# WISDEM/RAFT

Hardware: NVIDIA H100
Metric: RAO solves/sec (freq-bins x cases x designs) (higher is better)
Workload: dtype f64

## Files before the change

raft_b200/csrc/raftk.cu:

```cuda
#include <cuda_runtime.h>
#include <cooperative_groups.h>
#include <math_constants.h>
#include <stdint.h>
#include <stdio.h>
#include <stdlib.h>
#include <string.h>
#include <mutex>
#include <algorithm>
#include <type_traits>
#include <vector>

#include "../../include/raftk.h"

namespace cg = cooperative_groups;

static thread_local char g_err[512] = "";
static long long g_launches = 0;

static int set_err(int code, const char *fmt, const char *a = "", const char *b = "")
{
    snprintf(g_err, sizeof(g_err), fmt, a, b);
    return code;
}
#define CUDA_TRY(expr)                                                                          \
// ... 430 lines not shown
    CUDA_TRY(cudaOccupancyMaxActiveClusters(&clusters, k_rao_fused2<false>, &cfg));
    CUDA_TRY(cudaOccupancyMaxActiveBlocksPerMultiprocessor(&per_sm, k_rao_fused2<true>, F2_T, pl.smem));
    resident = per_sm * sm_count();
    std::lock_guard<std::mutex> lk(g_f2_occ_mu);
    g_f2_occ.push_back(F2Occ{dev, units, pl.CS, pl.smem, clusters, resident});
    return RAFTK_OK;
}

static int f2_pick_grid(const SolvePlan &pl, int units, bool &grid)
{
    grid = false;
    const char *x = getenv("RAFTK_FUSED2_XCHG");
    const bool force_c = x && !strcmp(x, "cluster"), force_g = x && !strcmp(x, "grid");
    if (x && *x && !force_c && !force_g) return set_err(RAFTK_EINVAL, "RAFTK_FUSED2_XCHG must be 'cluster' or 'grid', not '%s'", x);
    if (pl.CS <= 1 || force_c) return RAFTK_OK;
    int clusters = 0, resident = 0;
    if (int rc = f2_occupancy(pl, units, clusters, resident)) return rc;
    const bool fits = pl.xslots && (size_t)units * pl.CS <= (size_t)resident;
    if (force_g && !fits) return set_err(RAFTK_EINVAL, "RAFTK_FUSED2_XCHG=grid: the launch's CTAs cannot all be resident at once");
    grid = fits && (force_g || clusters < units);
    return RAFTK_OK;
}

static int run_fused2(const raftk_designs *d, const raftk_cases *c, const raftk_solve_opts *o, const raftk_outputs *out,
                      const SolvePlan &pl, void *workspace, cudaStream_t st, const raftk_peers *peers)
{
    prof_begin_call();
    DesignsDev D = to_dev(d, d->max_nodes, d->max_members);
    CasesDev C = to_dev(c);
    char *ws = static_cast<char *>(workspace);
    FusedParams P = fused_params(d, c, o, out, pl, peers);
    P.F0g = reinterpret_cast<double2 *>(ws);
    P.Eg = reinterpret_cast<double2 *>(ws + pl.o_E);
    P.Ag = reinterpret_cast<double2 *>(ws + pl.o_A);
    double *plan = reinterpret_cast<double *>(ws + pl.o_plan);
    P.plan = plan; P.plan_stride = pl.blob;
    if (!(o->flags & RAFTK_SOLVE_REUSE_PLAN)) {
        ProfScope ps(st, 0);
        const size_t psm = (3 * (size_t)d->max_nodes + d->max_members) * sizeof(double) + 2 * (size_t)d->max_members * sizeof(int);
        k_fused_plan<<<d->n_designs, 128, psm, st>>>(D, plan, pl.blob, pl.maxW, pl.maxH, pl.maxZ, pl.nwl);
        g_launches++;
    }
    const int units = d->n_designs * c->n_cases;
    bool grid = false;
    if (int rc = f2_pick_grid(pl, units, grid)) return rc;
    CUDA_TRY(grid ? g_f2_opt_grid.ensure(k_rao_fused2<true>, pl.smem) : g_f2_opt_cluster.ensure(k_rao_fused2<false>, pl.smem));
    cudaLaunchConfig_t cfg;
    cudaLaunchAttribute at;
    cluster_config(cfg, at, (size_t)units * pl.CS, F2_T, pl.smem, pl.CS, st);
    if (grid) {
        at.id = cudaLaunchAttributeCooperative;
        at.val.cooperative = 1;
        P.xrow = reinterpret_cast<double *>(ws + pl.o_xrow);
        P.xcnt = reinterpret_cast<unsigned *>(ws + pl.o_xcnt);
    }
    const int nphase = c->primary ? 2 : 1;
    if (c->primary) P.lin_g = reinterpret_cast<double *>(ws + pl.o_lin);
    for (int phase = 0; phase < nphase; phase++) {
        P.phase = c->primary ? phase : -1;
        {
            ProfScope ps(st, 2);
            if (grid) {
                CUDA_TRY(cudaMemsetAsync(P.xcnt, 0, (size_t)units * sizeof(unsigned), st));
                CUDA_TRY(cudaLaunchKernelEx(&cfg, k_rao_fused2<true>, D, C, P));
            } else {
                CUDA_TRY(cudaLaunchKernelEx(&cfg, k_rao_fused2<false>, D, C, P));
            }
        }
        g_launches++;
    }
    disp_launch(RAFTK_FAMILY_SOLVE, grid ? RAFTK_KERNEL_FUSED2_GRID : RAFTK_KERNEL_FUSED2_CLUSTER, F2_T, pl.CS, pl.nwl);
    g_disp.trains = c->primary != nullptr;
    CUDA_TRY(cudaGetLastError());
    return RAFTK_OK;
}

#ifdef RAFTK_F2_WAVE_TRACE
extern "C" int raftk_f2_trace_read(unsigned long long *host, int n_cta)
{
    if (n_cta < 0 || n_cta > F2_TRACE_MAX) return set_err(RAFTK_EINVAL, "n_cta must be in [0, F2_TRACE_MAX]");
    CUDA_TRY(cudaMemcpyFromSymbol(host, g_f2_trace, (size_t)n_cta * 3 * sizeof(unsigned long long)));
    return RAFTK_OK;
}
extern "C" int raftk_f2_occupancy(const raftk_designs *d, int n_cases, int cluster_size, int out[5])
{
    const SolvePlan pl = plan_solve(d, n_cases, cluster_size, WS_UNBOUNDED);
    if (pl.kind != SOLVE_FUSED2) return set_err(RAFTK_EINVAL, "not a k_rao_fused2 shape");
    const int units = d->n_designs * n_cases;
    int clusters = 0, resident = 0;
    bool grid = false;
    if (int rc = f2_occupancy(pl, units, clusters, resident)) return rc;
    if (int rc = f2_pick_grid(pl, units, grid)) return rc;
    out[0] = clusters; out[1] = resident; out[2] = grid ? 1 : 0; out[3] = pl.CS; out[4] = (int)pl.smem;
    return RAFTK_OK;
}
#endif

static int run_tables(const raftk_designs *d, const raftk_cases *c, const raftk_solve_opts *o, const raftk_outputs *out,
                      const double *Xi_in, int mode , const SolvePlan &pl,
                      void *workspace, size_t wbytes, cudaStream_t st)
{
    if (c->primary && mode != 2) return set_err(RAFTK_EINVAL, "cases.primary is only supported by raftk_solve_dynamics_*");
    const int nD = d->n_designs, nC = c->n_cases, nw = d->nw, per = pl.per;
    const bool excitation = mode != 1;
    if (excitation) prof_begin_call();
    DesignsDev D = to_dev(d, d->max_nodes, d->max_members);
    CasesDev C = to_dev(c);
    if (!workspace || wbytes < chunk_bytes(1, nC, d->max_nodes, nw)) return set_err(RAFTK_ENOMEM, "workspace smaller than one design's tables");
    if (mode == 1 && per < nD)
        return set_err(RAFTK_ENOMEM, "linearization needs the whole batch's tables resident in the workspace");
    if (mode != 2) {
        if (pl.smem > 227 * 1024) return set_err(RAFTK_EINVAL, "shared-memory plan exceeds 227 KB (nw per CTA too large)");
        static SmemOptIn opt;
        CUDA_TRY(opt.ensure(k_drag_solve, pl.smem));
// ... 1151 lines not shown
```

raft_b200/csrc/raftk_fused.cuh:

```cuda
#pragma once

struct FusedParams {
    int n_iter, CS, nwl, maxW, maxH, maxZ;
    double tol, xi_start;
    double2 *Xi_out, *Fdrag_out, *Finer_out, *Fbem_out;
    double2 *Xilast_out;
    const double2 *Xi_init;
    double *Bdrag_out, *zeta_out;
    int *status;
    double2 *F0g;
    double *lin_g;
    int phase;
    const double *plan; size_t plan_stride;
    double2 *Eg, *Ag;
    double *xrow; unsigned *xcnt;
    int n_peers, peer_rank;
    double2 *peer_Xi[RAFTK_MAX_PEERS];
    int *peer_status[RAFTK_MAX_PEERS];
};

#define IMEM_STRIDE 6
#define NCOEF 5

struct FSmem {
    double *mem, *node, *coef, *msum, *mat, *warp_part, *sums, *tot, *xi, *f0, *ckpt, *wkey, *hkey, *zkey, *scr, *trans;
    double2 *ebase, *abase, *wtab, *htab;
    int *imem, *node_w, *node_h, *cnt;
};

template <int NC>
__device__ __forceinline__ int warp_step_class(double *keys, int &n, int maxn, double x, double y, double tol, int &over)
{
    const int lane = threadIdx.x & 31;
    for (int b = 0; b < n; b += 32) {
        const int c = b + lane;
        const bool hit = c < n && fabs(keys[NC * c] - x) <= tol && (NC == 1 || fabs(keys[NC * c + NC - 1] - y) <= tol);
        const unsigned m = __ballot_sync(0xffffffffu, hit);
        if (m) return b + __ffs(m) - 1;
    }
    if (n == maxn) { over = 1; return 0; }
    if (lane == 0) { keys[NC * n] = x; if (NC == 2) keys[NC * n + NC - 1] = y; }
    __syncwarp();
    return n++;
}

__device__ __forceinline__ void step_classes_warp(const double *kx, const double *ky, const double *kz, int Ns, const double *z0,
                                               int z0_stride, int Nm, int maxW, int maxH, int maxZ, int nwl, double *wkey,
// ... 578 lines not shown
```

raft_b200/csrc/raftk_fused2.cuh:

```cuda
#pragma once

#define F2_T 128
#define F2_TRW 8

struct PlanLayout {
    int o_mem, o_node, nstr, o_mat, o_wkey, o_hkey, o_zkey, o_int, total;
    int i_imem, i_nodew, i_nodeh, i_nodem, i_cnt, i_chunk, n_int;
};

__host__ __device__ inline PlanLayout plan_layout(int NmP, int NsP, int maxW, int maxH, int maxZ)
{
    PlanLayout L;
    int p = 0;
    L.o_mem = p; p += NmP * MEM_STRIDE;
    L.nstr = (NsP + 1) & ~1;
    L.o_node = p; p += 8 * L.nstr;
    L.o_mat = p; p += 108;
    L.o_wkey = p; p += 2 * maxW;
    L.o_hkey = p; p += maxH;
    L.o_zkey = p; p += maxZ;
    p = (p + 1) & ~1;
    L.o_int = p;
    int q = 0;
    L.i_imem = q; q += NmP * IMEM_STRIDE;
// ... 77 lines not shown
            kx = fr[0] * step; ky = fr[1] * step; kz = fr[2] * step;
        }
        scr[j] = kx; scr[NsP + j] = ky; scr[2 * NsP + j] = kz;
    }
    __syncthreads();
    if (tid < 32)
        step_classes_warp(scr, scr + NsP, scr + 2 * NsP, Ns, z0s, 1, Nm, maxW, maxH, maxZ, nwl, wkey, hkey, zkey, node_w, node_h, imem, cnt);
    for (int j = Ns + tid; j < NsP + 12; j += T) { node_w[j] = maxW * nwl; node_h[j] = maxH * nwl; node_m[j] = Nm > 0 ? Nm - 1 : 0; }
    {
        int *chunk_g = ib + L.i_chunk;
        const int nchunk = (NsP + CHUNK_NODES - 1) / CHUNK_NODES;
        for (int ch = tid; ch < nchunk; ch += T) {
            unsigned cm = 0, slots = 0;
            for (int jj = 0; jj < CHUNK_NODES; jj++) {
                const int j = ch * CHUNK_NODES + jj;
                if (j >= Ns) break;
                const bool q = D.node_cd_q[nbase + j] != 0.0;
                const bool p = D.node_cd_p1[nbase + j] != 0.0 || D.node_cd_p2[nbase + j] != 0.0;
                cm |= ((q ? 1u : 0u) | (p ? 2u : 0u)) << (3 * jj);
                if (q || p) slots |= 1u << jj;
                if (p) slots |= 1u << (10 + jj);
                if (q && p) slots |= 1u << (20 + jj);
            }
            unsigned rm = 0;
            for (int rd = 0; rd < 4; rd++) if ((slots >> (rd * F2_TRW)) & 0xffu) rm |= 1u << rd;
            chunk_g[2 * ch] = (int)cm;
            chunk_g[2 * ch + 1] = (int)rm;
        }
    }
    __syncthreads();
    if (tid < 4) cnt_g[tid] = cnt[tid];
}

__device__ __forceinline__ unsigned smem_u32(const void *p) { return (unsigned)__cvta_generic_to_shared(p); }
__device__ __forceinline__ void mbar_init(unsigned long long *bar, unsigned count)
{
    asm volatile("mbarrier.init.shared::cta.b64 [%0], %1;" ::"r"(smem_u32(bar)), "r"(count) : "memory");
    asm volatile("fence.mbarrier_init.release.cluster;" ::: "memory");
}
__device__ __forceinline__ void mbar_expect_tx(unsigned long long *bar, unsigned bytes)
{
    asm volatile("mbarrier.arrive.expect_tx.shared::cta.b64 _, [%0], %1;" ::"r"(smem_u32(bar)), "r"(bytes) : "memory");
}
__device__ __forceinline__ void tma_bulk_g2s(void *dst, const void *src, unsigned bytes, unsigned long long *bar)
{
    asm volatile("cp.async.bulk.shared::cluster.global.mbarrier::complete_tx::bytes [%0], [%1], %2, [%3];"
                 ::"r"(smem_u32(dst)), "l"(src), "r"(bytes), "r"(smem_u32(bar)) : "memory");
}
__device__ __forceinline__ void mbar_wait(unsigned long long *bar, unsigned parity)
{
    asm volatile("{\n .reg .pred p;\n WAIT_%=:\n mbarrier.try_wait.parity.shared::cta.b64 p, [%0], %1;\n @p bra DONE_%=;\n bra WAIT_%=;\n DONE_%=:\n}"
                 ::"r"(smem_u32(bar)), "r"(parity) : "memory");
}

__device__ __noinline__ void sincos_once(double x, double *s, double *c) { sincos(x, s, c); }
__device__ __noinline__ double exp_once(double x) { return exp(x); }
__device__ __noinline__ double4 sincos2_once(double x0, double x1)
{
    double s0, c0, s1, c1;
    sincos(x0, &s0, &c0);
    sincos(x1, &s1, &c1);
    return make_double4(c0, s0, c1, s1);
}
__device__ __noinline__ double4 exp2pm_once(double a0, double a1) { return make_double4(exp(a0), exp(-a0), exp(a1), exp(-a1)); }
__device__ __noinline__ double4 depth2_once(double k0, double k1, double h, double z)
{
    double s0, c0, p0, s1, c1, p1;
    depth_funcs(k0, h, z, s0, c0, p0);
    depth_funcs(k1, h, z, s1, c1, p1);
    return make_double4(0.5 * (c0 + s0), 0.5 * (c0 - s0), 0.5 * (c1 + s1), 0.5 * (c1 - s1));
}
__device__ __noinline__ double jonswap_once(double w, double Hs, double Tp, double Gamma) { return jonswap(w, Hs, Tp, Gamma); }
__device__ __forceinline__ double zeta_f2(const CasesDev &Cs, int c, int i, int nw, double w, double dw)
{
    if (Cs.zeta_in) return Cs.zeta_in[(size_t)c * nw + i];
    const int spec = Cs.spec[c];
    double S = 0.0;
    if (spec == RAFTK_SPEC_JONSWAP) S = jonswap_once(w, Cs.Hs[c], Cs.Tp[c], Cs.gamma[c]);
    else if (spec == RAFTK_SPEC_UNIT) S = 1.0;
    else if (spec == RAFTK_SPEC_CONSTANT) S = Cs.Hs[c];
    return sqrt(2.0 * S * dw);
}
__device__ __noinline__ void depth_once(double k, double h, double z, double *S_, double *C_)
{
    double s, c, pd;
    depth_funcs(k, h, z, s, c, pd);
    *S_ = s; *C_ = c;
}

__host__ __device__ inline size_t fused2_smem_bytes(int Nm, int NsP, int nchunk, int nwl, int maxW, int maxH, int maxZ)
{
    const PlanLayout L = plan_layout(Nm, NsP, maxW, maxH, maxZ);
    const int nwarps = F2_T / 32;
    size_t dbl = (size_t)L.total + NCOEF * (size_t)NsP + (size_t)Nm * 8 + 36 + (size_t)nchunk * nwarps * 32 + 2 * ((size_t)nchunk * 32 + 2)
                 + (size_t)nchunk * 32 + (size_t)nwarps * F2_TRW * 33 + 2;
    dbl += 2 * ((size_t)(maxW + 1) + (maxH + 1)) * nwl + 12 * (size_t)nwl;
    return dbl * sizeof(double) + 64;
}

__device__ __forceinline__ bool conv_ok(double dr, double di, double xr, double xi, double tol)
{
    const double a = fma(dr, dr, di * di), b = fma(xr, xr, xi * xi);
    const double rhs = tol * (sqrt(b) + tol);
    return a < rhs * rhs;
}

#ifdef RAFTK_F2_WAVE_TRACE
#define F2_TRACE_MAX 4096
__device__ unsigned long long g_f2_trace[3 * F2_TRACE_MAX];
__device__ __forceinline__ unsigned long long f2_globaltimer()
{
    unsigned long long t;
    asm volatile("mov.u64 %0, %%globaltimer;" : "=l"(t));
    return t;
}
__device__ __forceinline__ void f2_trace(int slot)
{
    if (threadIdx.x != 0 || blockIdx.x >= F2_TRACE_MAX) return;
    unsigned smid;
    asm volatile("mov.u32 %0, %%smid;" : "=r"(smid));
    g_f2_trace[3 * blockIdx.x + slot] = f2_globaltimer();
    if (slot == 1) g_f2_trace[3 * blockIdx.x] = smid;
}
#define F2_TRACE(slot) f2_trace(slot)
#else
#define F2_TRACE(slot)
#endif

__device__ __forceinline__ int &f2_xchg_timeout()
{
    __shared__ int s_timeout;
    return s_timeout;
}

__device__ __forceinline__ void f2_xchg_arrive_wait(unsigned *cnt, unsigned target)
{
    __syncthreads();
    if (threadIdx.x == 0) {
        __threadfence();
        atomicAdd(cnt, 1u);
        const long long t0 = clock64();
        for (;;) {
            unsigned v;
            asm volatile("ld.acquire.gpu.global.u32 %0, [%1];" : "=r"(v) : "l"(cnt) : "memory");
            if (v >= target) break;
            if (clock64() - t0 > 4000000000LL) { f2_xchg_timeout() = RAFTK_FLAG_XCHG; break; }
        }
    }
    __syncthreads();
}

template <bool GRID>
__global__ void __launch_bounds__(F2_T, 2)
k_rao_fused2(DesignsDev D, CasesDev Cs, FusedParams P)
{
    F2_TRACE(1);
    extern __shared__ __align__(16) double smem_raw[];
    __shared__ __align__(8) unsigned long long mbar;
    constexpr int T = F2_T, nwarps = F2_T / 32;
    __shared__ int s_flw[nwarps];
    cg::cluster_group cluster = cg::this_cluster();
    const int CS = P.CS;
    const int rank = (CS > 1) ? (GRID ? (int)(blockIdx.x & (CS - 1)) : (int)cluster.block_rank()) : 0;
    const int unit = blockIdx.x / CS;
    const int d = unit / Cs.nC, c = unit % Cs.nC;
    const int nw = D.nw, tid = threadIdx.x, lane = tid & 31, warp = tid >> 5;
    const int prim = (P.phase >= 0 && Cs.primary) ? Cs.primary[c] : c;
    const bool secondary = prim != c;
    if ((P.phase == 0 && secondary) || (P.phase == 1 && !secondary)) return;

    const int NsP = D.max_nodes, NmP = D.max_members;
    const int nchunk = (NsP + CHUNK_NODES - 1) / CHUNK_NODES;
    const int nwl = P.nwl;
    const int f_begin = rank * nwl;
    const int nloc = max(0, min(nwl, nw - f_begin));
    const PlanLayout L = plan_layout(NmP, NsP, P.maxW, P.maxH, P.maxZ);

    double *blob = smem_raw;
    double *s_mem = blob + L.o_mem, *s_node = blob + L.o_node, *s_mat = blob + L.o_mat;
    const double *s_wkey = blob + L.o_wkey, *s_hkey = blob + L.o_hkey, *s_zkey = blob + L.o_zkey;
    const int *ib = reinterpret_cast<const int *>(blob + L.o_int);
    const int *s_imem = ib + L.i_imem, *s_nodew = ib + L.i_nodew, *s_nodeh = ib + L.i_nodeh, *s_nodem = ib + L.i_nodem, *s_cnt = ib + L.i_cnt;
    const int *s_chunk = ib + L.i_chunk;
    double *p = blob + L.total;
    double *s_coef = p; p += NCOEF * (size_t)NsP;
    double *s_msum = p; p += (size_t)NmP * 8;
    double *s_bmat = p; p += 36;
    double *s_wpart = p; p += (size_t)nchunk * nwarps * 32;
    double *s_sums = p; p += 2 * ((size_t)nchunk * 32 + 2);
    double *s_tot = p; p += (size_t)nchunk * 32;
    double *s_trans = p; p += (size_t)nwarps * F2_TRW * 33;
    p += ((p - smem_raw) & 1);
    double2 *s_wtab = reinterpret_cast<double2 *>(p); p += 2 * (size_t)(P.maxW + 1) * nwl;
    double2 *s_htab = reinterpret_cast<double2 *>(p); p += 2 * (size_t)(P.maxH + 1) * nwl;
    double *s_xi = p;
    const int sums_stride = nchunk * 32 + 2;
    const int nstr = L.nstr;
    const double *n_ls = s_node, *n_cdq = s_node + nstr, *n_cd1 = s_node + 2 * nstr, *n_cd2 = s_node + 3 * nstr;
    const double *n_inq = s_node + 4 * nstr, *n_in1 = s_node + 5 * nstr, *n_in2 = s_node + 6 * nstr, *n_pa = s_node + 7 * nstr;

    if (tid == 0) mbar_init(&mbar, 1);
    if (GRID && tid == 0) f2_xchg_timeout() = 0;
    __syncthreads();
    if (tid == 0) {
        const unsigned bytes = (unsigned)L.total * 8u;
        mbar_expect_tx(&mbar, bytes);
        tma_bulk_g2s(blob, P.plan + (size_t)d * P.plan_stride, bytes, &mbar);
    }
    const double beta = Cs.beta_deg[c] * (CUDART_PI / 180.0);
    double sb, cb;
    sincos(beta, &sb, &cb);
    mbar_wait(&mbar, 0);
    const int m0 = D.member_offset[d], Nm = D.member_offset[d + 1] - m0;
    const int nbase = D.mem_node_start[m0];
    const int Ns = D.mem_node_start[m0 + Nm] - nbase;
    for (int m = tid; m < Nm; m += T) {
        double *o = s_mem + m * MEM_STRIDE;
        for (int v = 0; v < 3; v++) o[18 + v] = o[3 * v] * cb + o[3 * v + 1] * sb;
    }
    __syncthreads();
    const int nW = s_cnt[0], nH = s_cnt[1], nZ = s_cnt[3];
    const bool plan_overflow = s_cnt[2] != 0;
    for (int t = tid; t < nchunk * nwarps * 32; t += T) s_wpart[t] = 0.0;

    const size_t ogl = ((size_t)d * Cs.nC + c) * 6 * nw;
    double2 *Eg = P.Eg + ((size_t)d * Cs.nC + c) * (size_t)NmP * nw;
    double2 *Ag = P.Ag + ((size_t)d * Cs.nC + c) * (size_t)P.maxZ * nw;

    const bool ok0 = tid < nloc, ok1 = tid + T < nloc;
    const int t0 = ok0 ? tid : 0, t1 = ok1 ? tid + T : t0;
    const int ibase = nloc > 0 ? f_begin : 0;
    const int i0 = ibase + t0, i1 = ibase + t1;
    const double w0 = ok0 ? D.w[i0] : 0.0, w1 = ok1 ? D.w[i1] : 0.0;
    const double2 *wtA = s_wtab + t0, *wtB = s_wtab + t1, *htA = s_htab + t0, *htB = s_htab + t1;
    const double2 zero2 = make_double2(0.0, 0.0);

    if (!plan_overflow && ok0) {
        const double kA = D.k[i0], kB = D.k[i1];
        const double zetaA = zeta_f2(Cs, c, i0, nw, D.w[i0], D.dw);
        const double zetaB = ok1 ? zeta_f2(Cs, c, i1, nw, D.w[i1], D.dw) : 0.0;
        if (P.zeta_out && d == 0) { P.zeta_out[(size_t)c * nw + i0] = zetaA; if (ok1) P.zeta_out[(size_t)c * nw + i1] = zetaB; }
        const double zwA = zetaA * w0, zwB = zetaB * w1;
#pragma unroll 1
        for (int x = 0; x < nW; x++) {
            const double g = s_wkey[2 * x] * cb + s_wkey[2 * x + 1] * sb;
            const double4 v = sincos2_once(-(kA * g), -(kB * g));
            s_wtab[x * nwl + t0] = make_double2(v.x, v.y);
            if (ok1) s_wtab[x * nwl + t1] = make_double2(v.z, v.w);
        }
#pragma unroll 1
        for (int x = 0; x < nH; x++) {
            const double4 v = exp2pm_once(kA * s_hkey[x], kB * s_hkey[x]);
            s_htab[x * nwl + t0] = make_double2(v.x, v.y);
            if (ok1) s_htab[x * nwl + t1] = make_double2(v.z, v.w);
        }
        s_wtab[P.maxW * nwl + t0] = make_double2(1.0, 0.0);
        s_htab[P.maxH * nwl + t0] = make_double2(1.0, 1.0);
        if (ok1) { s_wtab[P.maxW * nwl + t1] = make_double2(1.0, 0.0); s_htab[P.maxH * nwl + t1] = make_double2(1.0, 1.0); }
#pragma unroll 1
        for (int x = 0; x < nZ; x++) {
            const double4 v = depth2_once(kA, kB, D.depth, s_zkey[x]);
            Ag[(size_t)x * nw + i0] = make_double2(v.x, v.y);
            if (ok1) Ag[(size_t)x * nw + i1] = make_double2(v.z, v.w);
        }
#pragma unroll 1
        for (int m = 0; m < Nm; m++) {
            const double *o = s_mem + m * MEM_STRIDE;
            const double g = cb * o[22] + sb * o[23];
            const double4 v = sincos2_once(-(kA * g), -(kB * g));
            Eg[(size_t)m * nw + i0] = make_double2(zwA * v.x, zwA * v.y);
            if (ok1) Eg[(size_t)m * nw + i1] = make_double2(zwB * v.z, zwB * v.w);
        }
#pragma unroll
        for (int a = 0; a < 6; a++) {
            if (P.Xi_init) {
                const double2 x0 = P.Xi_init[ogl + (size_t)a * nw + i0];
                s_xi[(2 * a) * nwl + t0] = x0.x; s_xi[(2 * a + 1) * nwl + t0] = x0.y;
                if (ok1) { const double2 x1 = P.Xi_init[ogl + (size_t)a * nw + i1]; s_xi[(2 * a) * nwl + t1] = x1.x; s_xi[(2 * a + 1) * nwl + t1] = x1.y; }
            } else {
                s_xi[(2 * a) * nwl + t0] = P.xi_start; s_xi[(2 * a + 1) * nwl + t0] = 0.0;
                if (ok1) { s_xi[(2 * a) * nwl + t1] = P.xi_start; s_xi[(2 * a + 1) * nwl + t1] = 0.0; }
            }
        }
    }

    if (!plan_overflow) {
        const double kA = D.k[i0], kB = D.k[i1];
        const bool deepA = kA * D.depth > 89.4, deepB = kB * D.depth > 89.4;
        const double thA = tanh(kA * D.depth), thB = tanh(kB * D.depth);
        double FrA[6], FiA[6], FrB[6], FiB[6];
#pragma unroll
        for (int a = 0; a < 6; a++) { FrA[a] = 0.0; FiA[a] = 0.0; FrB[a] = 0.0; FiB[a] = 0.0; }
        const bool mcf = D.node_in_p1_w != nullptr;
        for (int m = 0; m < Nm; m++) {
            const double *o = s_mem + m * MEM_STRIDE;
            const int j0 = s_imem[IMEM_STRIDE * m], j1 = s_imem[IMEM_STRIDE * m + 1], zc = s_imem[IMEM_STRIDE * m + 4];
            const double ls0 = n_ls[j0];
            const double2 eA = ok0 ? Eg[(size_t)m * nw + i0] : zero2, eB = ok1 ? Eg[(size_t)m * nw + i1] : zero2;
            const double2 aA = Ag[(size_t)zc * nw + i0], aB = Ag[(size_t)zc * nw + i1];
            double erA = eA.x, eiA = eA.y, apA = aA.x, amA = aA.y, erB = eB.x, eiB = eB.y, apB = aB.x, amB = aB.y;
            const double hq = o[18], h1 = o[19], h2 = o[20];
            double AqrA = 0, AqiA = 0, A1rA = 0, A1iA = 0, A2rA = 0, A2iA = 0, L1rA = 0, L1iA = 0, L2rA = 0, L2iA = 0;
            double AqrB = 0, AqiB = 0, A1rB = 0, A1iB = 0, A2rB = 0, A2iB = 0, L1rB = 0, L1iB = 0, L2rB = 0, L2iB = 0;
            for (int j = j0; j < j1; j++) {
                const int ow = s_nodew[j], oh = s_nodeh[j];
                const double2 WA = wtA[ow], HA = htA[oh], WB = wtB[ow], HB = htB[oh];
                { const double tr = fma(erA, WA.x, -eiA * WA.y); eiA = fma(erA, WA.y, eiA * WA.x); erA = tr; }
                { const double tr = fma(erB, WB.x, -eiB * WB.y); eiB = fma(erB, WB.y, eiB * WB.x); erB = tr; }
                apA *= HA.x; amA *= HA.y; apB *= HB.x; amB *= HB.y;
                const double inq = n_inq[j], pa = n_pa[j], in1 = n_in1[j], in2 = n_in2[j], ls = n_ls[j];
                if (!mcf && inq == 0.0 && in1 == 0.0 && in2 == 0.0 && pa == 0.0) continue;
#define F2_F0_NODE(ER, EI, AP, AM, WW, KK, II, TH, DEEP, AQR, AQI, A1R, A1I, A2R, A2I, L1R, L1I, L2R, L2I)                     \
    {                                                                                                                             \
        double i1r = in1, i1i = 0.0, i2r = in2, i2i = 0.0;                                                                        \
        if (mcf) {                                                                                                                \
            const size_t jg = (size_t)(nbase + j);                                                                                \
            const double2 v1 = D.node_in_p1_w[jg * nw + II], v2 = D.node_in_p2_w[jg * nw + II];                                   \
            i1r = v1.x; i1i = v1.y; i2r = v2.x; i2i = v2.y;                                                                        \
        }                                                                                                                         \
        const double Cc = AP + AM, Sc = AP - AM;                                                                                  \
        double cr, ci;                                                                                                            \
        proj(ER, EI, Cc, Sc, hq, o[2], cr, ci);                                                                                   \
        double fqr = -WW * inq * ci, fqi = WW * inq * cr;                                                                         \
        proj(ER, EI, Cc, Sc, h1, o[5], cr, ci);                                                                                   \
        const double f1r = -WW * (i1r * ci + i1i * cr), f1i = WW * (i1r * cr - i1i * ci);                                         \
        proj(ER, EI, Cc, Sc, h2, o[8], cr, ci);                                                                                   \
        const double f2r = -WW * (i2r * ci + i2i * cr), f2i = WW * (i2r * cr - i2i * ci);                                         \
        if (pa != 0.0 && WW != 0.0) {                                                                                             \
            double Pd = Cc * TH;                                                                                                  \
            if (DEEP) Pd = Cc + exp_once(-KK * (o[21] + (ls - ls0) * o[2] + 2.0 * D.depth));                                      \
            const double sc = pa * Pd / WW;                                                                                       \
            fqr = fma(sc, ER, fqr); fqi = fma(sc, EI, fqi);                                                                       \
// ... 24 lines not shown
            double Fr[6], Fi[6];
#pragma unroll
            for (int a = 0; a < 6; a++) { Fr[a] = bsel == 0 ? FrA[a] : FrB[a]; Fi[a] = bsel == 0 ? FiA[a] : FiB[a]; }
            if (P.Finer_out)
                for (int a = 0; a < 6; a++) P.Finer_out[ogl + (size_t)a * nw + i] = make_double2(Fr[a], Fi[a]);
            if (D.n_bem_head > 0) {
                const double k = D.k[i], w = D.w[i];
                const double zeta = zeta_f2(Cs, c, i, nw, w, D.dw);
                double Br[6], Bi[6];
                bem_excitation(D, d, i, k, beta, sb, cb, zeta, Br, Bi);
#pragma unroll
                for (int a = 0; a < 6; a++) {
                    if (P.Fbem_out) P.Fbem_out[ogl + (size_t)a * nw + i] = make_double2(Br[a], Bi[a]);
                    Fr[a] += Br[a]; Fi[a] += Bi[a];
                }
            } else if (P.Fbem_out) {
                for (int a = 0; a < 6; a++) P.Fbem_out[ogl + (size_t)a * nw + i] = make_double2(0.0, 0.0);
            }
            if (Cs.F_2nd) {
#pragma unroll
                for (int a = 0; a < 6; a++) Fr[a] += Cs.F_2nd[ogl + (size_t)a * nw + i];
            }
#pragma unroll
            for (int a = 0; a < 6; a++) P.F0g[ogl + (size_t)a * nw + i] = make_double2(Fr[a], Fi[a]);
        }
    }
    if (plan_overflow) {
        for (int t = tid; t < nloc; t += T)
            for (int a = 0; a < 6; a++) P.Xi_out[ogl + (size_t)a * nw + f_begin + t] = make_double2(0.0, 0.0);
        if (P.Xilast_out)
            for (int t = tid; t < 6 * nloc; t += T) P.Xilast_out[ogl + (size_t)(t / nloc) * nw + f_begin + t % nloc] = make_double2(0.0, 0.0);
    }
    __syncthreads();

    const double *Aw = D.A_w ? D.A_w + (size_t)d * 36 * nw : nullptr;
    const double *Bw = D.B_w ? D.B_w + (size_t)d * 36 * nw : nullptr;
    int passes = 0, converged = 0, flags = plan_overflow ? RAFTK_FLAG_PLAN : 0, par = 0;
#define F2_XROW (P.xrow + (size_t)(blockIdx.x / CS) * 2 * CS * sums_stride)
#define F2_XCNT (P.xcnt + blockIdx.x / CS)
    const int max_pass = plan_overflow ? 0 : (secondary ? 1 : P.n_iter + 1);
    const size_t lin_stride = (size_t)NCOEF * NsP + 36;
    if (secondary && !plan_overflow) {
        const double *src = P.lin_g + ((size_t)d * Cs.nC + prim) * lin_stride;
#pragma unroll 1
        for (int t = tid; t < NCOEF * NsP; t += T) s_coef[t] = src[t];
#pragma unroll 1
        for (int t = tid; t < 36; t += T) s_bmat[t] = src[NCOEF * NsP + t];
        __syncthreads();
    }


    for (int it = 0; it < max_pass; it++) {
        if (!secondary) {
        double erA = 0, eiA = 0, apA = 0, amA = 0, erB = 0, eiB = 0, apB = 0, amB = 0;
        double mqrA = 0, mqiA = 0, m1rA = 0, m1iA = 0, m2rA = 0, m2iA = 0, u1rA = 0, u1iA = 0, u2rA = 0, u2iA = 0;
        double mqrB = 0, mqiB = 0, m1rB = 0, m1iB = 0, m2rB = 0, m2iB = 0, u1rB = 0, u1iB = 0, u2rB = 0, u2iB = 0;
        for (int ch = 0; ch < nchunk; ch++) {
            double acc[32];
#pragma unroll
            for (int t = 0; t < 32; t++) acc[t] = 0.0;
            const int jc0 = ch * CHUNK_NODES;
            const unsigned cmask = (unsigned)s_chunk[2 * ch], rmask = (unsigned)s_chunk[2 * ch + 1];
            if (jc0 < Ns) {
                int jj = 0;
                while (jj < CHUNK_NODES && jc0 + jj < Ns) {
                    const int jfirst = jc0 + jj;
// ... 1 lines not shown
                    const int mstart = s_imem[IMEM_STRIDE * mcur], jlast = s_imem[IMEM_STRIDE * mcur + 1] - jc0;
                    const double *o = s_mem + mcur * MEM_STRIDE;
#define F2_MEMBER_PROJ(TT, WW, OKK, MQR, MQI, M1R, M1I, M2R, M2I, U1R, U1I, U2R, U2I)                                          \
    {                                                                                                                             \
        double xr[6], xi[6];                                                                                                      \
        _Pragma("unroll") for (int a = 0; a < 6; a++) {                                                                           \
            xr[a] = OKK ? s_xi[(2 * a) * nwl + TT] : 0.0; xi[a] = OKK ? s_xi[(2 * a + 1) * nwl + TT] : 0.0;                      \
        }                                                                                                                         \
        double sr, si;                                                                                                            \
        sr = o[0] * xr[0] + o[1] * xr[1] + o[2] * xr[2] + o[9] * xr[3] + o[10] * xr[4] + o[11] * xr[5];                           \
        si = o[0] * xi[0] + o[1] * xi[1] + o[2] * xi[2] + o[9] * xi[3] + o[10] * xi[4] + o[11] * xi[5];                           \
        MQR = WW * si; MQI = -WW * sr;                                                                                            \
        sr = o[3] * xr[0] + o[4] * xr[1] + o[5] * xr[2] + o[12] * xr[3] + o[13] * xr[4] + o[14] * xr[5];                          \
        si = o[3] * xi[0] + o[4] * xi[1] + o[5] * xi[2] + o[12] * xi[3] + o[13] * xi[4] + o[14] * xi[5];                          \
        M1R = WW * si; M1I = -WW * sr;                                                                                            \
        sr = o[6] * xr[0] + o[7] * xr[1] + o[8] * xr[2] + o[15] * xr[3] + o[16] * xr[4] + o[17] * xr[5];                          \
        si = o[6] * xi[0] + o[7] * xi[1] + o[8] * xi[2] + o[15] * xi[3] + o[16] * xi[4] + o[17] * xi[5];                          \
        M2R = WW * si; M2I = -WW * sr;                                                                                            \
        sr = o[3] * xr[3] + o[4] * xr[4] + o[5] * xr[5];                                                                          \
        si = o[3] * xi[3] + o[4] * xi[4] + o[5] * xi[5];                                                                          \
        U1R = WW * si; U1I = -WW * sr;                                                                                            \
        sr = o[6] * xr[3] + o[7] * xr[4] + o[8] * xr[5];                                                                          \
        si = o[6] * xi[3] + o[7] * xi[4] + o[8] * xi[5];                                                                          \
        U2R = WW * si; U2I = -WW * sr;                                                                                            \
    }
                    if (jfirst == mstart) {
                        F2_MEMBER_PROJ(t0, w0, ok0, mqrA, mqiA, m1rA, m1iA, m2rA, m2iA, u1rA, u1iA, u2rA, u2iA)
                        F2_MEMBER_PROJ(t1, w1, ok1, mqrB, mqiB, m1rB, m1iB, m2rB, m2iB, u1rB, u1iB, u2rB, u2iB)
                    }
#undef F2_MEMBER_PROJ
                    const double hq = o[18], h1 = o[19], h2 = o[20], dzq = o[2], dz1 = o[5], dz2 = o[8];
                    if (jfirst == mstart) {
                        const int zc = s_imem[IMEM_STRIDE * mcur + 4];
                        const double2 eA = ok0 ? Eg[(size_t)mcur * nw + i0] : zero2, aA = Ag[(size_t)zc * nw + i0];
                        const double2 eB = ok1 ? Eg[(size_t)mcur * nw + i1] : zero2, aB = Ag[(size_t)zc * nw + i1];
                        erA = eA.x; eiA = eA.y; apA = aA.x; amA = aA.y;
                        erB = eB.x; eiB = eB.y; apB = aB.x; amB = aB.y;
                    }
#define F2_STEP_BIN(ER, EI, AP, AM, CW, CH, CC, SC)                                                                              \
    { const double tr = fma(ER, CW.x, -EI * CW.y); EI = fma(ER, CW.y, EI * CW.x); ER = tr; }                                      \
    AP *= CH.x; AM *= CH.y;                                                                                                       \
    const double CC = AP + AM, SC = AP - AM;
#define F2_SQ(ER, EI, CC, SC, HH, DZ, MR, MI, OUT)                                                                                \
    { double ar_, ai_; proj_add(ER, EI, CC, SC, HH, DZ, MR, MI, ar_, ai_); OUT = fma(ar_, ar_, ai_ * ai_); }
#define F2_P1_NODE(JJ, CWA, CHA, CWB, CHB, CL, NWA, NHA, NWB, NHB, NL)                                                           \
    {                                                                                                                             \
        const int jn = jc0 + JJ + 1;                                                                                              \
        const int ow = s_nodew[jn], oh = s_nodeh[jn];                                                                             \
        NWA = wtA[ow]; NHA = htA[oh]; NWB = wtB[ow]; NHB = htB[oh]; NL = n_ls[jn];                                                \
        const double ls = CL;                                                                                                     \
        F2_STEP_BIN(erA, eiA, apA, amA, CWA, CHA, CcA, ScA)                                                                       \
        F2_STEP_BIN(erB, eiB, apB, amB, CWB, CHB, CcB, ScB)                                                                       \
        const bool has_p = (cmask & (2u << (3 * JJ))) != 0u;                                                                      \
        if (has_p) {                                                                                                              \
            double pA, rA_, pB, rB_;                                                                                              \
            F2_SQ(erA, eiA, CcA, ScA, h1, dz1, fma(ls, u2rA, m1rA), fma(ls, u2iA, m1iA), pA)                                      \
            F2_SQ(erB, eiB, CcB, ScB, h1, dz1, fma(ls, u2rB, m1rB), fma(ls, u2iB, m1iB), pB)                                      \
            F2_SQ(erA, eiA, CcA, ScA, h2, dz2, fma(-ls, u1rA, m2rA), fma(-ls, u1iA, m2iA), rA_)                                   \
            F2_SQ(erB, eiB, CcB, ScB, h2, dz2, fma(-ls, u1rB, m2rB), fma(-ls, u1iB, m2iB), rB_)                                   \
            acc[JJ] += pA + pB; acc[10 + JJ] += rA_ + rB_;                                                                        \
        }                                                                                                                         \
        if (cmask & (1u << (3 * JJ))) {                                                                                           \
            double qA, qB;                                                                                                        \
            F2_SQ(erA, eiA, CcA, ScA, hq, dzq, mqrA, mqiA, qA)                                                                    \
            F2_SQ(erB, eiB, CcB, ScB, hq, dzq, mqrB, mqiB, qB)                                                                    \
            if (has_p) acc[20 + JJ] += qA + qB; else acc[JJ] += qA + qB;                                                          \
        }                                                                                                                         \
    }
// ... 112 lines not shown
            double s = 0.0;
            for (int m = 0; m < Nm; m++) {
                const double *o = s_mem + m * MEM_STRIDE, *ms = s_msum + m * 8;
                const double vqa = a < 3 ? o[a] : o[9 + a - 3], vqb = b < 3 ? o[b] : o[9 + b - 3];
                const double v1a = a < 3 ? o[3 + a] : o[12 + a - 3], v1b = b < 3 ? o[3 + b] : o[12 + b - 3];
                const double v2a = a < 3 ? o[6 + a] : o[15 + a - 3], v2b = b < 3 ? o[6 + b] : o[15 + b - 3];
                const double u1a = a < 3 ? 0.0 : o[6 + a - 3], u1b = b < 3 ? 0.0 : o[6 + b - 3];
                const double u2a = a < 3 ? 0.0 : -o[3 + a - 3], u2b = b < 3 ? 0.0 : -o[3 + b - 3];
                s += ms[0] * vqa * vqb;
                s += ms[1] * v1a * v1b + ms[2] * (v1a * u1b + u1a * v1b) + ms[3] * u1a * u1b;
                s += ms[4] * v2a * v2b + ms[5] * (v2a * u2b + u2a * v2b) + ms[6] * u2a * u2b;
            }
            s_bmat[tid] = s_mat[36 + tid] + s;
            if (P.Bdrag_out && rank == 0) P.Bdrag_out[((size_t)d * Cs.nC + c) * 36 + tid] = s;
        }
        __syncthreads();
        if (P.lin_g && P.phase == 0 && rank == 0) {
            double *dst = P.lin_g + ((size_t)d * Cs.nC + c) * lin_stride;
#pragma unroll 1
            for (int t = tid; t < NCOEF * NsP; t += T) dst[t] = s_coef[t];
#pragma unroll 1
            for (int t = tid; t < 36; t += T) dst[NCOEF * NsP + t] = s_bmat[t];
        }
        }

        int conv_local = 1, nan_local = 0;
        const double *cq_ = s_coef, *c1_ = s_coef + NsP, *cl1_ = s_coef + 2 * NsP, *c2_ = s_coef + 3 * NsP, *cl2_ = s_coef + 4 * NsP;
        double brA[6], biA[6], brB[6], biB[6];
#pragma unroll
        for (int a = 0; a < 6; a++) { brA[a] = 0.0; biA[a] = 0.0; brB[a] = 0.0; biB[a] = 0.0; }
        {
            double2 eA = ok0 ? Eg[i0] : zero2, eB = ok1 ? Eg[i1] : zero2;
            int zc = s_imem[4];
            double2 aA = Ag[(size_t)zc * nw + i0], aB = Ag[(size_t)zc * nw + i1];
            for (int m = 0; m < Nm; m++) {
                const double *o = s_mem + m * MEM_STRIDE;
                const double hq = o[18], h1 = o[19], h2 = o[20], dzq = o[2], dz1 = o[5], dz2 = o[8];
                const int j0 = s_imem[IMEM_STRIDE * m], j1 = s_imem[IMEM_STRIDE * m + 1];
                double erA = eA.x, eiA = eA.y, apA = aA.x, amA = aA.y, erB = eB.x, eiB = eB.y, apB = aB.x, amB = aB.y;
                if (m + 1 < Nm) {
                    zc = s_imem[IMEM_STRIDE * (m + 1) + 4];
                    eA = ok0 ? Eg[(size_t)(m + 1) * nw + i0] : zero2; eB = ok1 ? Eg[(size_t)(m + 1) * nw + i1] : zero2;
                    aA = Ag[(size_t)zc * nw + i0]; aB = Ag[(size_t)zc * nw + i1];
                }
                double AqrA = 0, AqiA = 0, A1rA = 0, A1iA = 0, A2rA = 0, A2iA = 0, L1rA = 0, L1iA = 0, L2rA = 0, L2iA = 0;
                double AqrB = 0, AqiB = 0, A1rB = 0, A1iB = 0, A2rB = 0, A2iB = 0, L1rB = 0, L1iB = 0, L2rB = 0, L2iB = 0;
#pragma unroll 2
                for (int j = j0; j < j1; j++) {
                    const int ow = s_nodew[j], oh = s_nodeh[j];
                    const double2 WA = wtA[ow], HA = htA[oh], WB = wtB[ow], HB = htB[oh];
                    const double bq = cq_[j], b1 = c1_[j], lb1 = cl1_[j], b2 = c2_[j], lb2 = cl2_[j];
                    { const double tr = fma(erA, WA.x, -eiA * WA.y); eiA = fma(erA, WA.y, eiA * WA.x); erA = tr; }
                    { const double tr = fma(erB, WB.x, -eiB * WB.y); eiB = fma(erB, WB.y, eiB * WB.x); erB = tr; }
                    apA *= HA.x; amA *= HA.y; apB *= HB.x; amB *= HB.y;
                    const double CcA = apA + amA, ScA = apA - amA, CcB = apB + amB, ScB = apB - amB;
                    double crA, ciA, crB, ciB;
                    if (bq != 0.0) {
                        proj(erA, eiA, CcA, ScA, hq, dzq, crA, ciA); proj(erB, eiB, CcB, ScB, hq, dzq, crB, ciB);
                        AqrA = fma(bq, crA, AqrA); AqiA = fma(bq, ciA, AqiA); AqrB = fma(bq, crB, AqrB); AqiB = fma(bq, ciB, AqiB);
                    }
                    if (b1 != 0.0 || b2 != 0.0) {
                        proj(erA, eiA, CcA, ScA, h1, dz1, crA, ciA); proj(erB, eiB, CcB, ScB, h1, dz1, crB, ciB);
                        A1rA = fma(b1, crA, A1rA); A1iA = fma(b1, ciA, A1iA); L1rA = fma(lb1, crA, L1rA); L1iA = fma(lb1, ciA, L1iA);
                        A1rB = fma(b1, crB, A1rB); A1iB = fma(b1, ciB, A1iB); L1rB = fma(lb1, crB, L1rB); L1iB = fma(lb1, ciB, L1iB);
                        proj(erA, eiA, CcA, ScA, h2, dz2, crA, ciA); proj(erB, eiB, CcB, ScB, h2, dz2, crB, ciB);
                        A2rA = fma(b2, crA, A2rA); A2iA = fma(b2, ciA, A2iA); L2rA = fma(lb2, crA, L2rA); L2iA = fma(lb2, ciA, L2iA);
                        A2rB = fma(b2, crB, A2rB); A2iB = fma(b2, ciB, A2iB); L2rB = fma(lb2, crB, L2rB); L2iB = fma(lb2, ciB, L2iB);
                    }
                }
#pragma unroll
                for (int a = 0; a < 3; a++) {
                    brA[a] += o[a] * AqrA + o[3 + a] * A1rA + o[6 + a] * A2rA;
                    biA[a] += o[a] * AqiA + o[3 + a] * A1iA + o[6 + a] * A2iA;
                    brA[3 + a] += o[9 + a] * AqrA + o[12 + a] * A1rA + o[15 + a] * A2rA + o[6 + a] * L1rA - o[3 + a] * L2rA;
                    biA[3 + a] += o[9 + a] * AqiA + o[12 + a] * A1iA + o[15 + a] * A2iA + o[6 + a] * L1iA - o[3 + a] * L2iA;
                    brB[a] += o[a] * AqrB + o[3 + a] * A1rB + o[6 + a] * A2rB;
// ... 77 lines not shown
            double *xrow = F2_XROW;
            if (tid == 0) { double *mine = xrow + ((size_t)par * CS + rank) * sums_stride + nchunk * 32; mine[0] = (double)conv_all; mine[1] = (double)(nan_all | f2_xchg_timeout()); }
            f2_xchg_arrive_wait(F2_XCNT, (unsigned)(CS * (secondary ? it + 1 : 2 * it + 2)));
            int ca = 1, na = 0;
#pragma unroll 1
            for (int r0 = 0; r0 < CS; r0 += 4) {
                double fc[4], fn[4];
#pragma unroll
                for (int r = 0; r < 4; r++) {
                    const double *rem = xrow + ((size_t)par * CS + (r0 + r < CS ? r0 + r : 0)) * sums_stride + nchunk * 32;
                    fc[r] = __ldcg(rem); fn[r] = __ldcg(rem + 1);
                }
#pragma unroll
                for (int r = 0; r < 4; r++) { ca &= (int)fc[r]; na |= (int)fn[r]; }
            }
            conv_all = ca; nan_all = na;
        } else if (CS > 1) {
            if (tid == 0) { s_sums[par * sums_stride + nchunk * 32] = (double)conv_all; s_sums[par * sums_stride + nchunk * 32 + 1] = (double)nan_all; }
            cluster.sync();
            int ca = 1, na = 0;
#pragma unroll 1
            for (int r0 = 0; r0 < CS; r0 += 4) {
                double fc[4], fn[4];
#pragma unroll
                for (int r = 0; r < 4; r++) {
                    const double *rem = cluster.map_shared_rank(s_sums, r0 + r < CS ? r0 + r : 0) + par * sums_stride + nchunk * 32;
                    fc[r] = rem[0]; fn[r] = rem[1];
                }
#pragma unroll
                for (int r = 0; r < 4; r++) { ca &= (int)fc[r]; na |= (int)fn[r]; }
            }
            conv_all = ca; nan_all = na;
        }
        par ^= 1;
        flags |= nan_all;
        if (nan_all & (GRID ? RAFTK_FLAG_NAN | RAFTK_FLAG_XCHG : RAFTK_FLAG_NAN)) break;
        if (conv_all) { converged = 1; break; }
    }
    if (P.status && rank == 0 && tid == 0) {
        int *st = P.status + ((size_t)d * Cs.nC + c) * 4;
        st[0] = secondary ? 0 : passes; st[1] = secondary ? 1 : converged; st[2] = flags; st[3] = secondary ? prim + 1 : 0;
    }
    if (P.n_peers > 1) {
        for (int t = tid; t < nloc; t += T) {
            const int i = f_begin + t;
#pragma unroll
            for (int a = 0; a < 6; a++) {
                const size_t o_ = ogl + (size_t)a * nw + i;
                const double2 v = P.Xi_out[o_];
#pragma unroll 1
                for (int pr = 0; pr < P.n_peers; pr++)
                    if (pr != P.peer_rank) P.peer_Xi[pr][o_] = v;
            }
        }
        if (rank == 0 && tid == 0) {
            const size_t so = ((size_t)d * Cs.nC + c) * 4;
#pragma unroll 1
            for (int pr = 0; pr < P.n_peers; pr++)
                if (pr != P.peer_rank && P.peer_status[pr]) {
                    int *st = P.peer_status[pr] + so;
                    st[0] = secondary ? 0 : passes; st[1] = secondary ? 1 : converged; st[2] = flags; st[3] = secondary ? prim + 1 : 0;
                }
        }
    }
    if (!GRID && CS > 1) cluster.sync();
    F2_TRACE(2);
// ... 4 lines not shown
```

Before: 201.6 million.

## Hoist depth-function table into per-design precompute kernel shared across cases

The depth-dependent cosh/sinh table (Ag) is no longer computed by every (design, case) CTA inside the fused solve. A new k_fused_depth kernel fills it once per design during plan building, and the solve kernel reads it through a per-design pointer. This removes redundant transcendental work that was repeated for each case, at the cost of an extra launch and a read-only global table. The change also adds trace slots and a layout query helper for debugging.

```diff
diff --git a/raft_b200/csrc/raftk.cu b/raft_b200/csrc/raftk.cu
--- a/raft_b200/csrc/raftk.cu
+++ b/raft_b200/csrc/raftk.cu
@@ -486,14 +486,16 @@
     FusedParams P = fused_params(d, c, o, out, pl, peers);
     P.F0g = reinterpret_cast<double2 *>(ws);
     P.Eg = reinterpret_cast<double2 *>(ws + pl.o_E);
-    P.Ag = reinterpret_cast<double2 *>(ws + pl.o_A);
+    double2 *Ad = reinterpret_cast<double2 *>(ws + pl.o_A);
+    P.Ag = Ad;
     double *plan = reinterpret_cast<double *>(ws + pl.o_plan);
     P.plan = plan; P.plan_stride = pl.blob;
     if (!(o->flags & RAFTK_SOLVE_REUSE_PLAN)) {
         ProfScope ps(st, 0);
         const size_t psm = (3 * (size_t)d->max_nodes + d->max_members) * sizeof(double) + 2 * (size_t)d->max_members * sizeof(int);
         k_fused_plan<<<d->n_designs, 128, psm, st>>>(D, plan, pl.blob, pl.maxW, pl.maxH, pl.maxZ, pl.nwl);
-        g_launches++;
+        k_fused_depth<<<dim3((d->nw + 127) / 128, d->n_designs), 128, 0, st>>>(D, plan, pl.blob, Ad, pl.maxW, pl.maxH, pl.maxZ);
+        g_launches += 2;
     }
     const int units = d->n_designs * c->n_cases;
     bool grid = false;
@@ -529,11 +531,22 @@
     return RAFTK_OK;
 }
 
+extern "C" int raftk_f2_table_layout(const raftk_designs *d, int n_cases, int cluster_size, long long out[6])
+{
+    const SolvePlan pl = plan_solve(d, n_cases, cluster_size, WS_UNBOUNDED);
+    if (pl.kind != SOLVE_FUSED2) return set_err(RAFTK_EINVAL, "not a k_rao_fused2 shape");
+    const PlanLayout L = plan_layout(d->max_members, d->max_nodes, pl.maxW, pl.maxH, pl.maxZ);
+    const long long v[6] = {(long long)pl.o_plan, (long long)pl.blob * 8, (long long)pl.o_A, (long long)L.o_zkey * 8,
+                            (long long)L.o_int * 8 + 4LL * L.i_cnt, pl.maxZ};
+    for (int i = 0; i < 6; i++) out[i] = v[i];
+    return RAFTK_OK;
+}
+
 #ifdef RAFTK_F2_WAVE_TRACE
 extern "C" int raftk_f2_trace_read(unsigned long long *host, int n_cta)
 {
     if (n_cta < 0 || n_cta > F2_TRACE_MAX) return set_err(RAFTK_EINVAL, "n_cta must be in [0, F2_TRACE_MAX]");
-    CUDA_TRY(cudaMemcpyFromSymbol(host, g_f2_trace, (size_t)n_cta * 3 * sizeof(unsigned long long)));
+    CUDA_TRY(cudaMemcpyFromSymbol(host, g_f2_trace, (size_t)n_cta * F2_TRACE_SLOTS * sizeof(unsigned long long)));
     return RAFTK_OK;
 }
 extern "C" int raftk_f2_occupancy(const raftk_designs *d, int n_cases, int cluster_size, int out[5])
diff --git a/raft_b200/csrc/raftk_fused.cuh b/raft_b200/csrc/raftk_fused.cuh
--- a/raft_b200/csrc/raftk_fused.cuh
+++ b/raft_b200/csrc/raftk_fused.cuh
@@ -12,7 +12,8 @@
     double *lin_g;
     int phase;
     const double *plan; size_t plan_stride;
-    double2 *Eg, *Ag;
+    double2 *Eg;
+    const double2 *Ag;
     double *xrow; unsigned *xcnt;
     int n_peers, peer_rank;
     double2 *peer_Xi[RAFTK_MAX_PEERS];
diff --git a/raft_b200/csrc/raftk_fused2.cuh b/raft_b200/csrc/raftk_fused2.cuh
--- a/raft_b200/csrc/raftk_fused2.cuh
+++ b/raft_b200/csrc/raftk_fused2.cuh
@@ -133,6 +133,21 @@
     if (tid < 4) cnt_g[tid] = cnt[tid];
 }
 
+__global__ void __launch_bounds__(128) k_fused_depth(DesignsDev D, const double *plan, size_t stride, double2 *Ad, int maxW, int maxH, int maxZ)
+{
+    const int d = blockIdx.y, nw = D.nw, i = blockIdx.x * blockDim.x + threadIdx.x;
+    const PlanLayout L = plan_layout(D.max_members, D.max_nodes, maxW, maxH, maxZ);
+    const double *blob = plan + (size_t)d * stride;
+    const int *cnt = reinterpret_cast<const int *>(blob + L.o_int) + L.i_cnt;
+    if (i >= nw || cnt[2] != 0) return;
+    const double k = D.k[i];
+    for (int x = 0; x < cnt[3]; x++) {
+        double s, c, pd;
+        depth_funcs(k, D.depth, blob[L.o_zkey + x], s, c, pd);
+        Ad[((size_t)d * maxZ + x) * nw + i] = make_double2(0.5 * (c + s), 0.5 * (c - s));
+    }
+}
+
 __device__ __forceinline__ unsigned smem_u32(const void *p) { return (unsigned)__cvta_generic_to_shared(p); }
 __device__ __forceinline__ void mbar_init(unsigned long long *bar, unsigned count)
 {
@@ -164,13 +179,6 @@
     return make_double4(c0, s0, c1, s1);
 }
 __device__ __noinline__ double4 exp2pm_once(double a0, double a1) { return make_double4(exp(a0), exp(-a0), exp(a1), exp(-a1)); }
-__device__ __noinline__ double4 depth2_once(double k0, double k1, double h, double z)
-{
-    double s0, c0, p0, s1, c1, p1;
-    depth_funcs(k0, h, z, s0, c0, p0);
-    depth_funcs(k1, h, z, s1, c1, p1);
-    return make_double4(0.5 * (c0 + s0), 0.5 * (c0 - s0), 0.5 * (c1 + s1), 0.5 * (c1 - s1));
-}
 __device__ __noinline__ double jonswap_once(double w, double Hs, double Tp, double Gamma) { return jonswap(w, Hs, Tp, Gamma); }
 __device__ __forceinline__ double zeta_f2(const CasesDev &Cs, int c, int i, int nw, double w, double dw)
 {
@@ -208,7 +216,8 @@
 
 #ifdef RAFTK_F2_WAVE_TRACE
 #define F2_TRACE_MAX 4096
-__device__ unsigned long long g_f2_trace[3 * F2_TRACE_MAX];
+#define F2_TRACE_SLOTS 16
+__device__ unsigned long long g_f2_trace[F2_TRACE_SLOTS * F2_TRACE_MAX];
 __device__ __forceinline__ unsigned long long f2_globaltimer()
 {
     unsigned long long t;
@@ -220,12 +229,14 @@
     if (threadIdx.x != 0 || blockIdx.x >= F2_TRACE_MAX) return;
     unsigned smid;
     asm volatile("mov.u32 %0, %%smid;" : "=r"(smid));
-    g_f2_trace[3 * blockIdx.x + slot] = f2_globaltimer();
-    if (slot == 1) g_f2_trace[3 * blockIdx.x] = smid;
+    g_f2_trace[F2_TRACE_SLOTS * blockIdx.x + slot] = f2_globaltimer();
+    if (slot == 1) g_f2_trace[F2_TRACE_SLOTS * blockIdx.x] = smid;
 }
 #define F2_TRACE(slot) f2_trace(slot)
+#define F2_TRACE_PASS(it) f2_trace(6 + min((it), F2_TRACE_SLOTS - 7))
 #else
 #define F2_TRACE(slot)
+#define F2_TRACE_PASS(it)
 #endif
 
 __device__ __forceinline__ int &f2_xchg_timeout()
@@ -279,7 +290,7 @@
 
     double *blob = smem_raw;
     double *s_mem = blob + L.o_mem, *s_node = blob + L.o_node, *s_mat = blob + L.o_mat;
-    const double *s_wkey = blob + L.o_wkey, *s_hkey = blob + L.o_hkey, *s_zkey = blob + L.o_zkey;
+    const double *s_wkey = blob + L.o_wkey, *s_hkey = blob + L.o_hkey;
     const int *ib = reinterpret_cast<const int *>(blob + L.o_int);
     const int *s_imem = ib + L.i_imem, *s_nodew = ib + L.i_nodew, *s_nodeh = ib + L.i_nodeh, *s_nodem = ib + L.i_nodem, *s_cnt = ib + L.i_cnt;
     const int *s_chunk = ib + L.i_chunk;
@@ -300,6 +311,7 @@
     const double *n_ls = s_node, *n_cdq = s_node + nstr, *n_cd1 = s_node + 2 * nstr, *n_cd2 = s_node + 3 * nstr;
     const double *n_inq = s_node + 4 * nstr, *n_in1 = s_node + 5 * nstr, *n_in2 = s_node + 6 * nstr, *n_pa = s_node + 7 * nstr;
 
+    __shared__ const double2 *volatile s_Ag;
     if (tid == 0) mbar_init(&mbar, 1);
     if (GRID && tid == 0) f2_xchg_timeout() = 0;
     __syncthreads();
@@ -307,11 +319,13 @@
         const unsigned bytes = (unsigned)L.total * 8u;
         mbar_expect_tx(&mbar, bytes);
         tma_bulk_g2s(blob, P.plan + (size_t)d * P.plan_stride, bytes, &mbar);
+        s_Ag = P.Ag + (size_t)d * P.maxZ * nw;
     }
     const double beta = Cs.beta_deg[c] * (CUDART_PI / 180.0);
     double sb, cb;
     sincos(beta, &sb, &cb);
     mbar_wait(&mbar, 0);
+    F2_TRACE(3);
     const int m0 = D.member_offset[d], Nm = D.member_offset[d + 1] - m0;
     const int nbase = D.mem_node_start[m0];
     const int Ns = D.mem_node_start[m0 + Nm] - nbase;
@@ -320,13 +334,12 @@
         for (int v = 0; v < 3; v++) o[18 + v] = o[3 * v] * cb + o[3 * v + 1] * sb;
     }
     __syncthreads();
-    const int nW = s_cnt[0], nH = s_cnt[1], nZ = s_cnt[3];
+    const int nW = s_cnt[0], nH = s_cnt[1];
     const bool plan_overflow = s_cnt[2] != 0;
     for (int t = tid; t < nchunk * nwarps * 32; t += T) s_wpart[t] = 0.0;
 
     const size_t ogl = ((size_t)d * Cs.nC + c) * 6 * nw;
     double2 *Eg = P.Eg + ((size_t)d * Cs.nC + c) * (size_t)NmP * nw;
-    double2 *Ag = P.Ag + ((size_t)d * Cs.nC + c) * (size_t)P.maxZ * nw;
 
     const bool ok0 = tid < nloc, ok1 = tid + T < nloc;
     const int t0 = ok0 ? tid : 0, t1 = ok1 ? tid + T : t0;
@@ -358,12 +371,6 @@
         s_wtab[P.maxW * nwl + t0] = make_double2(1.0, 0.0);
         s_htab[P.maxH * nwl + t0] = make_double2(1.0, 1.0);
         if (ok1) { s_wtab[P.maxW * nwl + t1] = make_double2(1.0, 0.0); s_htab[P.maxH * nwl + t1] = make_double2(1.0, 1.0); }
-#pragma unroll 1
-        for (int x = 0; x < nZ; x++) {
-            const double4 v = depth2_once(kA, kB, D.depth, s_zkey[x]);
-            Ag[(size_t)x * nw + i0] = make_double2(v.x, v.y);
-            if (ok1) Ag[(size_t)x * nw + i1] = make_double2(v.z, v.w);
-        }
 #pragma unroll 1
         for (int m = 0; m < Nm; m++) {
             const double *o = s_mem + m * MEM_STRIDE;
@@ -384,6 +391,7 @@
             }
         }
     }
+    F2_TRACE(4);
 
     if (!plan_overflow) {
         const double kA = D.k[i0], kB = D.k[i1];
@@ -398,7 +406,7 @@
             const int j0 = s_imem[IMEM_STRIDE * m], j1 = s_imem[IMEM_STRIDE * m + 1], zc = s_imem[IMEM_STRIDE * m + 4];
             const double ls0 = n_ls[j0];
             const double2 eA = ok0 ? Eg[(size_t)m * nw + i0] : zero2, eB = ok1 ? Eg[(size_t)m * nw + i1] : zero2;
-            const double2 aA = Ag[(size_t)zc * nw + i0], aB = Ag[(size_t)zc * nw + i1];
+            const double2 aA = s_Ag[(size_t)zc * nw + i0], aB = s_Ag[(size_t)zc * nw + i1];
             double erA = eA.x, eiA = eA.y, apA = aA.x, amA = aA.y, erB = eB.x, eiB = eB.y, apB = aB.x, amB = aB.y;
             const double hq = o[18], h1 = o[19], h2 = o[20];
             double AqrA = 0, AqiA = 0, A1rA = 0, A1iA = 0, A2rA = 0, A2iA = 0, L1rA = 0, L1iA = 0, L2rA = 0, L2iA = 0;
@@ -489,6 +497,7 @@
             for (int t = tid; t < 6 * nloc; t += T) P.Xilast_out[ogl + (size_t)(t / nloc) * nw + f_begin + t % nloc] = make_double2(0.0, 0.0);
     }
     __syncthreads();
+    F2_TRACE(5);
 
     const double *Aw = D.A_w ? D.A_w + (size_t)d * 36 * nw : nullptr;
     const double *Bw = D.B_w ? D.B_w + (size_t)d * 36 * nw : nullptr;
@@ -556,8 +565,8 @@
                     const double hq = o[18], h1 = o[19], h2 = o[20], dzq = o[2], dz1 = o[5], dz2 = o[8];
                     if (jfirst == mstart) {
                         const int zc = s_imem[IMEM_STRIDE * mcur + 4];
-                        const double2 eA = ok0 ? Eg[(size_t)mcur * nw + i0] : zero2, aA = Ag[(size_t)zc * nw + i0];
-                        const double2 eB = ok1 ? Eg[(size_t)mcur * nw + i1] : zero2, aB = Ag[(size_t)zc * nw + i1];
+                        const double2 eA = ok0 ? Eg[(size_t)mcur * nw + i0] : zero2, aA = s_Ag[(size_t)zc * nw + i0];
+                        const double2 eB = ok1 ? Eg[(size_t)mcur * nw + i1] : zero2, aB = s_Ag[(size_t)zc * nw + i1];
                         erA = eA.x; eiA = eA.y; apA = aA.x; amA = aA.y;
                         erB = eB.x; eiB = eB.y; apB = aB.x; amB = aB.y;
                     }
@@ -736,7 +745,7 @@
         {
             double2 eA = ok0 ? Eg[i0] : zero2, eB = ok1 ? Eg[i1] : zero2;
             int zc = s_imem[4];
-            double2 aA = Ag[(size_t)zc * nw + i0], aB = Ag[(size_t)zc * nw + i1];
+            double2 aA = s_Ag[(size_t)zc * nw + i0], aB = s_Ag[(size_t)zc * nw + i1];
             for (int m = 0; m < Nm; m++) {
                 const double *o = s_mem + m * MEM_STRIDE;
                 const double hq = o[18], h1 = o[19], h2 = o[20], dzq = o[2], dz1 = o[5], dz2 = o[8];
@@ -745,7 +754,7 @@
                 if (m + 1 < Nm) {
                     zc = s_imem[IMEM_STRIDE * (m + 1) + 4];
                     eA = ok0 ? Eg[(size_t)(m + 1) * nw + i0] : zero2; eB = ok1 ? Eg[(size_t)(m + 1) * nw + i1] : zero2;
-                    aA = Ag[(size_t)zc * nw + i0]; aB = Ag[(size_t)zc * nw + i1];
+                    aA = s_Ag[(size_t)zc * nw + i0]; aB = s_Ag[(size_t)zc * nw + i1];
                 }
                 double AqrA = 0, AqiA = 0, A1rA = 0, A1iA = 0, A2rA = 0, A2iA = 0, L1rA = 0, L1iA = 0, L2rA = 0, L2iA = 0;
                 double AqrB = 0, AqiB = 0, A1rB = 0, A1iB = 0, A2rB = 0, A2iB = 0, L1rB = 0, L1iB = 0, L2rB = 0, L2iB = 0;
@@ -889,6 +898,7 @@
             }
             conv_all = ca; nan_all = na;
         }
+        F2_TRACE_PASS(it);
         par ^= 1;
         flags |= nan_all;
         if (nan_all & (GRID ? RAFTK_FLAG_NAN | RAFTK_FLAG_XCHG : RAFTK_FLAG_NAN)) break;
```

After: 207.5 million, median of 6. 1.03x the previous value.
